# Gadersd/stable-diffusion-xl-burn

Measured on AMD Instinct MI355X. Metric: images/sec SDXL-base 1024x1024 30-step CFG7.5 (whole job); UNet step ms p50, higher is better.
Workload: dtype f16; 1 GPU; SDXL-base 1024x1024, n_steps=30 (31 CFG UNet step pairs), CFG 7.5, batch 1 prompt/GPU + VAE decode to u8 (BASELINE configs[1]); precision=f16, vae_dtype=f32_split, weights=synthetic seeded (random-init SDXL-base architecture), mix_classes=0, parallelism=replica x1, 1 prompt per GPU, weights broadcast once over RCCL, hipgraph=True, split_cfg=False, fused_xattn=True, pipelined_decode=False, prompts_per_call=1, full=False, library=stable-diffusion-xl-burn_amd/lib/libsdxl_mi355.so, debug_set=

## Files before the change

### stable-diffusion-xl-burn_amd/csrc/igemm_wreg.hip

```cpp
#include "igemm_common.h"
#include <atomic>

namespace sdxl {

template <int OFF> __device__ __forceinline__ half8 wreg_gload128(const half_t* ptr) {
  half8 v;
  asm volatile("global_load_dwordx4 %0, %1, off offset:%2" : "=v"(v) : "v"(ptr), "n"(OFF));
  return v;
}

__global__ void repack_wfrag_kernel(const f32x4* __restrict__ src, f32x4* __restrict__ dst, int nblocks, int nk) {
  const size_t i = (size_t)blockIdx.x * blockDim.x + threadIdx.x;
  const size_t total = (size_t)nblocks * nk * 256;
  if (i >= total) return;
  const int lane = (int)(i & 63), kk = (int)((i >> 6) & 3);
  const size_t t = i >> 8;
  const int kt = (int)(t % nk);
  const int nb = (int)(t / nk);
  dst[i] = src[(size_t)(nb * 32 + (lane & 31)) * (nk * 8) + kt * 8 + kk * 2 + (lane >> 5)];
}
void launch_repack_wfrag(const void* w, void* wf, int Npad, int Kpad, hipStream_t s) {
  const int nblocks = Npad / 32, nk = Kpad / 64;
  const size_t total = (size_t)nblocks * nk * 256;
  hipLaunchKernelGGL(repack_wfrag_kernel, dim3((unsigned)((total + 255) / 256)), dim3(256), 0, s, reinterpret_cast<const f32x4*>(w),
                     reinterpret_cast<f32x4*>(wf), nblocks, nk);
}

template <int TM> struct WregEpiOperands { half8 rh[TM]; f32x4 rf[TM][2]; f32x4 bz0, bz1, sg0, sg1; };
template <int TM>
__device__ __forceinline__ void wreg_epilogue_request(const IgemmParams& p, int mw, int nw, int lane, int t, const void* zeros, WregEpiOperands<TM>& op) {
  const int fr = lane & 31, fh = lane >> 5;
  const f32x4* zv = reinterpret_cast<const f32x4*>(zeros);
  const int n0 = nw + t * 16 + 8 * fh;
  const bool r16 = p.R && p.r_dt == DT_F16, r32 = p.R && p.r_dt == DT_F32;
#pragma unroll
  for (int i = 0; i < TM; ++i) {
    const int m = mw + i * 32 + fr;
    const bool ok = m < p.M;
    const size_t o = (size_t)(ok ? m : 0) * p.ldr + n0;
    op.rh[i] = *((r16 && ok) ? reinterpret_cast<const half8*>(reinterpret_cast<const half_t*>(p.R) + o) : reinterpret_cast<const half8*>(zeros));
    if (r32) {
      op.rf[i][0] = *(ok ? reinterpret_cast<const f32x4*>(reinterpret_cast<const float*>(p.R) + o) : zv);
      op.rf[i][1] = *(ok ? reinterpret_cast<const f32x4*>(reinterpret_cast<const float*>(p.R) + o + 4) : zv);
    }
  }
  op.bz0 = *(p.bias ? reinterpret_cast<const f32x4*>(p.bias + nw + 16 * t + 4 * fh) : zv);
  op.bz1 = *(p.bias ? reinterpret_cast<const f32x4*>(p.bias + nw + 16 * t + 8 + 4 * fh) : zv);
  op.sg0 = *(p.shadow ? reinterpret_cast<const f32x4*>(p.shadow_gamma + n0) : zv);
  op.sg1 = *(p.shadow ? reinterpret_cast<const f32x4*>(p.shadow_gamma + n0 + 4) : zv);
}
template <int TM>
__device__ __forceinline__ void wreg_epilogue(const IgemmParams& p, const f32x16 (&acc)[TM], int mw, int nw, int lane, int w, int t,
                                              float* xch, const WregEpiOperands<TM>& op) {
  const int fr = lane & 31, fh = lane >> 5;
  float sv[TM][8];
  int m[TM];
  bool mok[TM];
#pragma unroll
  for (int i = 0; i < TM; ++i) { m[i] = mw + i * 32 + fr; mok[i] = m[i] < p.M; }
  const int n0 = nw + t * 16 + 8 * fh;
  {
    const bool r16 = p.R && p.r_dt == DT_F16, r32 = p.R && p.r_dt == DT_F32;
    const half8 (&rh)[TM] = op.rh;
    const f32x4 (&rf)[TM][2] = op.rf;
    const f32x4 bz0 = op.bz0, bz1 = op.bz1;
#pragma unroll
    for (int i = 0; i < TM; ++i) {
      f32x4 v0, v1;
#pragma unroll
      for (int r = 0; r < 4; ++r) {
        v0[r] = t ? acc[i][8 + r] : acc[i][r];
        v1[r] = t ? acc[i][12 + r] : acc[i][4 + r];
      }
      v0 = v0 + bz0; v1 = v1 + bz1;
      float wv[8];
#pragma unroll
      for (int r = 0; r < 4; ++r) {
        const auto sw = __builtin_amdgcn_permlane32_swap(__float_as_uint(v0[r]), __float_as_uint(v1[r]), false, false);
        wv[r] = __uint_as_float(sw[0]);
        wv[4 + r] = __uint_as_float(sw[1]);
      }
      if (r16) {
#pragma unroll
        for (int e = 0; e < 8; ++e) wv[e] += (float)rh[i][e];
      } else if (r32) {
#pragma unroll
        for (int e = 0; e < 4; ++e) { wv[e] += rf[i][0][e]; wv[4 + e] += rf[i][1][e]; }
      }
      if (p.c_dt == DT_F16) {
        half8 h;
#pragma unroll
        for (int e = 0; e < 8; ++e) h[e] = (half_t)wv[e];
        if (mok[i]) *reinterpret_cast<half8*>(reinterpret_cast<half_t*>(p.C) + (size_t)m[i] * p.ldc + n0) = h;
#pragma unroll
        for (int e = 0; e < 8; ++e) sv[i][e] = (float)h[e];
      } else {
        if (mok[i]) {
          float* cp = reinterpret_cast<float*>(p.C) + (size_t)m[i] * p.ldc + n0;
          *reinterpret_cast<f32x4*>(cp) = f32x4{wv[0], wv[1], wv[2], wv[3]};
          *reinterpret_cast<f32x4*>(cp + 4) = f32x4{wv[4], wv[5], wv[6], wv[7]};
        }
        if (p.shadow && p.shadow_lo_scale < 0.f) {
          float xs[8];
#pragma unroll
          for (int e = 0; e < 4; ++e) { xs[e] = wv[e] * op.sg0[e]; xs[4 + e] = wv[4 + e] * op.sg1[e]; }
          if (mok[i]) store_hl8(reinterpret_cast<float*>(p.shadow) + (size_t)m[i] * p.shadow_ld, n0, xs);
        } else
        if (p.shadow) {
          half8 hs;
#pragma unroll
          for (int e = 0; e < 4; ++e) { hs[e] = (half_t)(wv[e] * op.sg0[e]); hs[4 + e] = (half_t)(wv[4 + e] * op.sg1[e]); }
          if (p.shadow_lo_scale > 0.f) {
            half8 hl;
#pragma unroll
            for (int e = 0; e < 4; ++e) {
              float x0 = wv[e] * op.sg0[e], x1 = wv[4 + e] * op.sg1[e];
              asm("" : "+v"(x0)); asm("" : "+v"(x1));
// ... 137 lines not shown
    xattn_unit_long(qf, op.kf, op.vf, fx, p.xa_nctx, fh, o);
  } else
  xattn_unit(qf, op.kf, op.vf, p.xa_nctx, fh, o);
  const int m = m0 + 32 * ui + fr;
  half_t* crow = reinterpret_cast<half_t*>(p.C) + (size_t)(m < p.M ? m : 0) * p.ldc + n0 + 64 * uh + 8 * fh;
#pragma unroll
  for (int dt = 0; dt < 2; ++dt)
#pragma unroll
    for (int t = 0; t < 2; ++t) {
      half8 h;
#pragma unroll
      for (int r = 0; r < 4; ++r) {
        const auto sw = __builtin_amdgcn_permlane32_swap(__float_as_uint(o[dt][8 * t + r]), __float_as_uint(o[dt][8 * t + 4 + r]), false, false);
        h[r] = (half_t)__uint_as_float(sw[0]);
        h[4 + r] = (half_t)__uint_as_float(sw[1]);
      }
      if (m < p.M) *reinterpret_cast<half8*>(crow + 32 * dt + 16 * t) = h;
    }
}

#ifdef SDXL_MEASURE
__device__ unsigned* g_wreg_tl = nullptr;
void igemm_set_wreg_timeline(void* buf) {
  unsigned* b = reinterpret_cast<unsigned*>(buf);
  if (hipMemcpyToSymbol(HIP_SYMBOL(g_wreg_tl), &b, sizeof(b)) != hipSuccess) throw std::runtime_error("igemm_wreg: cannot set the timeline buffer");
}
#define WREG_STAMP(i) do { wtl[i] = (unsigned)__builtin_amdgcn_s_memtime(); } while (0)
#else
#define WREG_STAMP(i) do { } while (0)
#endif
constexpr int wreg_mode_flags(int m) {
  return m >= 16 ? m : m == 1 ? 16 : m == 2 ? 32 : m == 3 ? 64 : m == 4 ? 128 : m == 5 ? 256 : m == 6 ? 512 : m == 7 ? 1024 : m == 8 ? 2048 : 0;
}
template <int BM, int L, int MODE = 0, int XA = 0>
__global__ __launch_bounds__(512) void igemm_wreg_kernel(const IgemmParams p, const void* zeros) {
#ifdef SDXL_MEASURE
  unsigned wtl[8] = {0, 0, 0, 0, 0, 0, 0, 0};
  wtl[6] = (unsigned)__builtin_amdgcn_s_memrealtime();
#endif
  WREG_STAMP(0);
  kernarg_prefetch<(int)sizeof(IgemmParams) + 8>();
  constexpr int NG = 2;
  constexpr int NSG = L + 1;
  constexpr int TM = BM / 32;
  constexpr int PP = BM / 32;
  constexpr int FL = wreg_mode_flags(MODE);
  constexpr bool NOMFMA = FL & 16, FROZEN = FL & 32, NOVMEM = FL & 64, NOBAR = FL & 128, XCDALT = FL & 256, NOA = FL & 512, NOWL = FL & 1024,
                 ACONTIG = FL & 2048, NOLDS = FL & 4096;
  constexpr int NW = NOWL ? 0 : 4;
  constexpr int NA = NOA ? 0 : PP;
  constexpr int U = NA + NW;
  constexpr int NOPS = U;
  constexpr int SLOT = BM * 128;
  constexpr int RING = NSG * SLOT;
  constexpr int KSTEP = 64 * NG;
  static_assert(BM % 32 == 0 && TM >= 2 && TM <= 4, "wave tile: 64 / 96 / 128 rows");
  static_assert((NSG - 1) * SLOT + (TM - 1) * 4096 < 65536, "fragment offsets must fit the ds_read immediate");
  static_assert(PP + (L - 1) * U < 64 && L >= 2, "vmcnt is 6 bits");
  static_assert(NOPS <= 3 * TM, "one VMEM operation per MFMA gap before the rendezvous");
  extern __shared__ __attribute__((aligned(16))) char smem[];
  const unsigned lds0 = (unsigned)(uintptr_t)(lptr_t)smem;

  const int tid = threadIdx.x, lane = tid & 63;
  const int wave = __builtin_amdgcn_readfirstlane(tid >> 6);
  const int g = wave >> 2, w = wave & 3;

  const int tilesM = (p.M + BM - 1) / BM;
  const int nwg = tilesM * (p.N >> 7);
  if ((int)blockIdx.x >= nwg) {
#pragma unroll
    for (int r = 0; r < 3; ++r)
      if (p.warm[r]) igemm_warm_body<512>(p.warm[r], p.warm_bytes[r], (int)blockIdx.x - nwg, (int)gridDim.x - nwg);
    return;
  }
  int bid = blockIdx.x;
  {
    const int q = nwg >> 3, r = nwg & 7, xcd = bid & 7, idx = bid >> 3;
    bid = (xcd < r ? xcd * (q + 1) : r * (q + 1) + (xcd - r) * q) + idx;
  }
  const int tilesN = p.N >> 7;
  int tm = bid / tilesN, tn = bid - tm * tilesN;
  if constexpr (XCDALT) { tn = bid / tilesM; tm = bid - tn * tilesM; }
  if (p.wreg_xcd2d && !(tilesM & 1) && !(tilesN & 1) && tilesN >= 8) {
    const int ch = tilesN >> 1, prow = tilesM >> 1, ptiles = prow * ch;
    const int patch = bid / ptiles, idx = bid - patch * ptiles;
    const int r = idx / ch;
    tm = (patch >> 1) * prow + r;
    tn = (patch & 1) * ch + (idx - r * ch);
  }
  const int m0 = tm * BM, n0 = tn * 128;
  const int nk = p.Kpad >> 6;
  const int nkg = (nk - g + 1) >> 1;

  const half_t* wp = reinterpret_cast<const half_t*>(p.Wf) + ((size_t)((n0 >> 5) + w) * nk + g) * 2048 + lane * 8;
  half8 Wr[NSG][4];
  if constexpr (NOVMEM || NOWL) { static_for<NSG>([&](auto S_) { static_for<4>([&](auto K_) { Wr[decltype(S_)::value][decltype(K_)::value] = half8{1, 1, 1, 1, 1, 1, 1, 1}; }); }); }
  auto loadW = [&](auto S, auto KK) {
    constexpr int s = decltype(S)::value, kk = decltype(KK)::value;
    if constexpr (!NOVMEM && !NOWL) Wr[s][kk] = wreg_gload128<kk * 1024>(wp);
    if constexpr (kk == 3 && !FROZEN) wp += NG * 2048;
  };
  const half_t* Ag = reinterpret_cast<const half_t*>(p.A);
  const half_t* aptr[PP];
  int aadv[PP];
  char* const ring = smem + g * RING;
  auto setupA = [&]() {
#pragma unroll
    for (int q = 0; q < PP; ++q) {
      const int row = (q * 4 + w) * 8 + (lane >> 3);
      const int m = m0 + row;
      const bool ok = m < p.M;
      aptr[q] = ok ? Ag + (size_t)m * p.lda + g * 64 + (((lane & 7) ^ ((row >> 1) & 7)) << 3) : reinterpret_cast<const half_t*>(zeros);
      aadv[q] = ok ? KSTEP : 0;
      if constexpr (ACONTIG) {
        aptr[q] = Ag + ((size_t)(tm % (p.M / BM)) * nk + g) * (BM * 64) + (q * 4 + w) * 512 + lane * 8;
        aadv[q] = NG * BM * 64;
      }
    }
  };
  auto pieceA = [&](auto S, auto Q) {
    constexpr int s = decltype(S)::value, q = decltype(Q)::value;
    if constexpr (!NOVMEM && !NOA) __builtin_amdgcn_global_load_lds((gptr_t)aptr[q], (lptr_t)(ring + s * SLOT + (q * 4 + w) * 1024), 16, 0, 0);
    if constexpr (!FROZEN) aptr[q] += aadv[q];
  };
  auto vmem_op = [&](auto S, auto X) {
    constexpr int x = decltype(X)::value;
    if constexpr (x < NW) loadW(S, X);
    else pieceA(S, std::integral_constant<int, x - NW>{});
  };

  const int fr = lane & 31, fh = lane >> 5;
  unsigned fa[4];
  {
    const unsigned basea = lds0 + g * RING + fr * 128 + ((fh ^ ((fr >> 1) & 7)) << 4);
#pragma unroll
    for (int kk = 0; kk < 4; ++kk) fa[kk] = basea ^ (kk << 5);
  }
  half8 fA[2][TM];
  if constexpr (NOLDS) { static_for<TM>([&](auto I) { fA[0][decltype(I)::value] = fA[1][decltype(I)::value] = half8{1, 1, 1, 1, 1, 1, 1, 1}; }); }
  auto ldsA = [&](auto SET, auto S, auto KK) {
    constexpr int set = decltype(SET)::value, s = decltype(S)::value, kk = decltype(KK)::value;
    if constexpr (!NOLDS) static_for<TM>([&](auto I) { fA[set][decltype(I)::value] = lds_read128<s * SLOT + decltype(I)::value * 4096>(fa[kk]); });
  };
  using I0 = std::integral_constant<int, 0>; using I1 = std::integral_constant<int, 1>;
  using I2 = std::integral_constant<int, 2>; using I3 = std::integral_constant<int, 3>;

  const int s0 = ((L - (nkg - 1)) % NSG + NSG) % NSG;
  const int ns = nkg > L ? nkg - L : 0;

  static_for<NSG>([&](auto C) {
    constexpr int c = decltype(C)::value;
    if (s0 == c && nkg > 0) static_for<4>([&](auto KK) { loadW(C, KK); });
  });
  setupA();
  static_for<NSG>([&](auto C) {
    constexpr int c = decltype(C)::value;
    if (s0 == c) {
      static_for<L>([&](auto I) {
        constexpr int i = decltype(I)::value;
        using SI = std::integral_constant<int, (c + i) % NSG>;
        if (i < nkg) {
          if constexpr (i > 0) static_for<4>([&](auto KK) { loadW(SI{}, KK); });
          static_for<PP>([&](auto Q) { pieceA(SI{}, Q); });
        }
      });
    }
  });
  __builtin_amdgcn_sched_barrier(0);
  WREG_STAMP(1);
  f32x16 acc[TM];
#pragma unroll
  for (int i = 0; i < TM; ++i)
#pragma unroll
    for (int r = 0; r < 16; ++r) acc[i][r] = 0.f;

// ... 43 lines not shown
      wait_lgkmcnt<0>();
      if constexpr (!NOBAR) __builtin_amdgcn_s_barrier();
      asm volatile("" ::: "memory");
      __builtin_amdgcn_sched_barrier(0);
      ldsA(I0{}, SN{}, I0{});
    } else {
      wait_lgkmcnt<0>();
    }
    mma(I1{}, S, I3{}, SF{}, NOX{});
  };
  using STEADY = std::integral_constant<int, 0>;
  if (ns > 0) {
    const int first = s0 == 0 ? 1 : NSG - s0 + 1;
    static_for<L>([&](auto C) { constexpr int c = decltype(C)::value + 1; if (s0 != 0 && s0 <= c) ktile(std::integral_constant<int, c>{}, STEADY{}); });
    ktile(I0{}, STEADY{});
    for (int pass = (ns - first) / NSG; pass > 0; --pass) {
      static_for<L>([&](auto C) { ktile(std::integral_constant<int, decltype(C)::value + 1>{}, STEADY{}); });
      ktile(I0{}, STEADY{});
    }
  }
  static_for<L>([&](auto X) {
    constexpr int D = L - decltype(X)::value;
    if (D <= nkg) ktile(std::integral_constant<int, L + 1 - D>{}, std::integral_constant<int, D>{});
  });
  WREG_STAMP(3);
  if constexpr (!NOBAR) { if ((nk & 1) && g == 1) __builtin_amdgcn_s_barrier(); }
  asm volatile("" ::: "memory");
  __builtin_amdgcn_sched_barrier(0);

  WregEpiOperands<TM> eop;
  WregXaOperands<XA ? BM : 64> xop;
  float* const xa_coef = reinterpret_cast<float*>(smem + NG * RING);
  if constexpr (XA) { static_assert(MODE == 0, "production arithmetic only"); wreg_xattn_request<BM, XA == 2>(p, m0, n0, lane, wave, zeros, xop); }
  else wreg_epilogue_request<TM>(p, m0, n0 + w * 32, lane, g, zeros, eop);
  static_assert(4 * TM * 2 * 64 * 16 <= L * SLOT, "a group's four exchange pieces must fit its dead slots 0 .. L - 1");
  f32x4* xw = reinterpret_cast<f32x4*>(smem + g * RING) + (size_t)w * (TM * 2 * 64) + lane;
  const f32x4* xo = reinterpret_cast<const f32x4*>(smem + (1 - g) * RING) + (size_t)w * (TM * 2 * 64) + lane;
#pragma unroll
  for (int i = 0; i < TM; ++i)
#pragma unroll
    for (int qq = 0; qq < 2; ++qq) {
      f32x4 v;
#pragma unroll
      for (int r = 0; r < 4; ++r) v[r] = g ? acc[i][4 * qq + r] : acc[i][8 + 4 * qq + r];
      xw[(i * 2 + qq) * 64] = v;
    }
  if constexpr (XA) wreg_xattn_coef<BM>(p, m0, lane, wave, xop, xa_coef);
  wait_lgkmcnt<0>();
  __builtin_amdgcn_s_barrier();
  asm volatile("" ::: "memory");
#pragma unroll
  for (int i = 0; i < TM; ++i)
#pragma unroll
    for (int qq = 0; qq < 2; ++qq) {
      const f32x4 o = xo[(i * 2 + qq) * 64];
#pragma unroll
      for (int r = 0; r < 4; ++r) {
        if (g) acc[i][8 + 4 * qq + r] = o[r] + acc[i][8 + 4 * qq + r];
        else acc[i][4 * qq + r] = acc[i][4 * qq + r] + o[r];
      }
    }
  WREG_STAMP(4);
  static_assert((2 * BM + 6 * 2 * BM) * 4 <= SLOT, "statistics exchange must fit one slot");
  float* xch = reinterpret_cast<float*>(smem + L * SLOT);
  if constexpr (XA) wreg_xattn_tail<BM, L, XA == 2>(p, acc, m0, n0, lane, wave, smem, xa_coef, xop);
  else wreg_epilogue<TM>(p, acc, m0, n0 + w * 32, lane, w, g, xch, eop);
#ifdef SDXL_MEASURE
  WREG_STAMP(5);
  asm volatile("s_waitcnt vmcnt(0)" ::: "memory");
  wtl[7] = (unsigned)__builtin_amdgcn_s_memrealtime();
  { const unsigned t6 = (unsigned)__builtin_amdgcn_s_memtime();
    if (g_wreg_tl && lane == 0) { unsigned* d = g_wreg_tl + ((size_t)blockIdx.x * 8 + wave) * 16; for (int i = 0; i < 8; ++i) d[i] = wtl[i]; d[8] = t6; } }
#endif
}

static std::atomic<int> g_wreg_xcd2d{0};
void igemm_set_wreg_xcd2d(int v) { g_wreg_xcd2d = v; }
static std::atomic<int> g_warm_enable{1};
void igemm_set_warm(int v) { g_warm_enable = v; }
int igemm_warm_enabled() { return g_warm_enable.load(); }

template <int BM, int L, int MODE = 0, int XA = 0>
static void launch_wreg_t(const IgemmParams& p, const IgemmChoice& c, hipStream_t s) {
  constexpr size_t lds = (size_t)2 * (L + 1) * BM * 128 + (XA ? BM * 8 : 0);
  static_assert(lds >= (size_t)8 * (BM / 32) * 2048 + (size_t)(2 * BM + 6 * 2 * BM) * 4, "exchange areas must fit the dead rings");
  if ((size_t)c.lds != lds) throw std::logic_error("igemm_wreg: choice and kernel disagree on the LDS layout");
  set_max_dynamic_lds<&igemm_wreg_kernel<BM, L, MODE, XA>>(lds, igemm_current_device());
  IgemmParams q = p;
  q.wreg_xcd2d = g_wreg_xcd2d.load();
  hipLaunchKernelGGL((igemm_wreg_kernel<BM, L, MODE, XA>), dim3(c.grid), dim3(c.block), lds, s, q, igemm_zero_page());
}

void launch_igemm_wreg(const IgemmParams& p, const IgemmChoice& c, hipStream_t s) {
#define WREG(BM, L, MODE, XA) \
  if (c.bm == BM && c.ns == L && c.mode == (MODE) && (c.xa > 1 ? 2 : c.xa) == XA) return launch_wreg_t<BM, L, (MODE), XA>(p, c, s)
#ifdef SDXL_MEASURE
  WREG(96, 3, 0, 0); WREG(96, 4, 0, 0); WREG(128, 2, 0, 0);
  WREG(96, 2, 1, 0); WREG(96, 2, 2, 0); WREG(96, 2, 3, 0); WREG(96, 2, 4, 0); WREG(96, 2, 5, 0);
  WREG(96, 2, 6, 0); WREG(96, 2, 7, 0); WREG(96, 2, 8, 0);
  WREG(96, 2, 16 | 32, 0); WREG(96, 2, 16 | 32 | 4096, 0); WREG(96, 2, 16 | 32 | 4096 | 128, 0); WREG(96, 2, 16 | 4096, 0); WREG(96, 2, 4096, 0);
#endif
  WREG(64, 2, 0, 0); WREG(96, 2, 0, 0);
  WREG(64, 2, 0, 1); WREG(96, 2, 0, 1);
  WREG(64, 2, 0, 2); WREG(96, 2, 0, 2);
#undef WREG
  throw std::logic_error("igemm_wreg: the selection chose a kernel that is not instantiated");
}

}
```

### stable-diffusion-xl-burn_amd/csrc/select.cpp

```cpp
#include "kernels.h"
#include <algorithm>
#include <atomic>
#include <cstring>
#include <stdexcept>

namespace sdxl {

namespace {
struct KnobSlot { const char* key; int SelectKnobs::*field; };
constexpr KnobSlot kKnobSlots[] = {
    {"igemm_variant", &SelectKnobs::igemm_variant}, {"igemm_wreg", &SelectKnobs::igemm_wreg}, {"wreg_xattn", &SelectKnobs::wreg_xattn},
    {"hl_tile96", &SelectKnobs::hl_tile96},         {"igemm_tsw", &SelectKnobs::igemm_tsw},   {"wide_db", &SelectKnobs::wide_db},
    {"attn_variant", &SelectKnobs::attn_variant},   {"attn_xsplit", &SelectKnobs::attn_xsplit},
#ifdef SDXL_MEASURE
    {"igemm_unrolled", &SelectKnobs::igemm_unrolled},
#endif
};
constexpr int kNumKnobs = sizeof(kKnobSlots) / sizeof(kKnobSlots[0]);
struct KnobStore {
  std::atomic<int> v[kNumKnobs];
  KnobStore() { const SelectKnobs d; for (int i = 0; i < kNumKnobs; ++i) v[i] = d.*kKnobSlots[i].field; }
};
KnobStore g_knobs;
}
// ... 70 lines not shown
  if (p.ph_rows <= 0 || p.ph_wbytes == 0 || p.B <= 0 || p.ph_rows != p.B * p.Hin * p.Win || p.M != 4 * p.ph_rows) return false;
  if (p.ksize != 2 || p.stride != 1 || p.up != 0 || p.pad != 1 || p.Hout != p.Hin || p.Wout != p.Win) return false;
  if ((p.Hin * p.Win) % 128 != 0 || p.Cin % kt != 0 || p.K != 4 * p.Cin || p.Kpad != p.K) return false;
  return p.act == 0 && p.n_split >= p.N && !p.R && !p.ebias && !p.stat_out && !p.gn_part && !p.ln_stat && !p.xa_k && !p.shadow;
}
int pick_phase_tile(const IgemmParams& p, int nk, bool hl) {
  double best = 1e300;
  int number = 36;
  for (int n : {35, 36, 38, 49}) {
    const Tile& t = tile(n);
    if (p.ph_rows % t.bm != 0 || !tile_takes(t, p) || (hl && n == 38)) continue;
    const double cost = tile_cost(p.M, p.N, nk, t.bm, t.bn, t.w);
    if (cost < best) { best = cost; number = n; }
  }
  if (!hl && number == 36 && nk >= 40) number = 44;
  return number;
}

struct Fill { long t96, t128, t256; double eff128, eff256; };
Fill chip_fill(const IgemmParams& p) {
  const long cols = (p.N + 127) / 128;
  const long t96 = (long)((p.M + 95) / 96) * cols, t128 = (long)((p.M + 127) / 128) * cols, t256 = (long)((p.M + 255) / 256) * cols;
  return {t96, t128, t256, (double)t128 / (double)(((t128 + 255) / 256) * 256), (double)t256 / (double)(((t256 + 255) / 256) * 256)};
}
int fill_tile_256_or_128(const IgemmParams& p) {
  const Fill f = chip_fill(p);
  return f.eff256 >= f.eff128 ? 35 : 36;
}

bool wreg_pair_grid_fits(const IgemmParams& p) {
  const long rows = 2L * (p.rpb > 0 ? p.rpb : p.M);
  return ((rows + 95) / 96) * (long)(p.N / 128) <= 512;
}
int wreg_rows(const IgemmParams& p) { return (long)((p.M + 63) / 64) * (p.N / 128) <= 256 ? 64 : 96; }
bool wreg_takes(const IgemmParams& p, const SelectKnobs& k, bool xa) {
  if (!p.Wf || !k.zero_page || (xa ? !p.xa_k || p.xa_k_lo : p.xa_k != nullptr)) return false;
  if (p.a_dt != DT_F16 || (p.c_dt != DT_F16 && (xa || p.c_dt != DT_F32))) return false;
  if (p.ksize != 1 || p.stride != 1 || p.up != 0 || p.pad != 0 || p.Hin != p.Hout || p.Win != p.Wout) return false;
  if (p.N % 128 != 0 || p.Cin != p.K || p.K != p.Kpad || p.Kpad % 64 != 0 || p.Kpad < 128) return false;
  if (p.act != 0 || p.n_split < p.N || p.gn_part || p.acc_scale || p.ebias) return false;
  if ((p.lda & 7) != 0 || misaligned16(p.A) || (p.ldc & 7) != 0 || misaligned16(p.C)) return false;
  if (xa) {
    if (p.stat_out || p.R || p.shadow || p.rpb <= 0 || p.rpb % 64 != 0 || p.M % p.rpb != 0 || p.xa_nctx < 1) return false;
    return p.xa_nctx <= 96 || igemm_xattn_ok(p.a_dt, p.c_dt, p.M, p.N, p.K, p.rpb, p.xa_nctx, k, true);
  }
  if (p.ln_stat || (p.R && ((p.ldr & 7) != 0 || misaligned16(p.R)))) return false;
  if (p.shadow && (p.c_dt != DT_F32 || !p.shadow_gamma || (p.shadow_ld & (p.shadow_lo_scale < 0.f ? 15 : 7)) != 0 || misaligned16(p.shadow))) return false;
  return true;
}
#ifdef SDXL_MEASURE
struct WregForced { int number, bm, depth, mode; };
constexpr WregForced kWregForced[] = {{61, 128, 2, 0}, {63, 96, 2, 1}, {64, 96, 2, 2}, {65, 96, 2, 3}, {66, 96, 2, 4}, {67, 96, 2, 5}, {68, 96, 3, 0},
    {69, 96, 4, 0}, {70, 96, 2, 6}, {71, 96, 2, 7}, {72, 96, 2, 8}, {73, 96, 2, 16 | 32}, {74, 96, 2, 16 | 32 | 4096}, {75, 96, 2, 16 | 32 | 4096 | 128},
    {76, 96, 2, 16 | 4096}, {77, 96, 2, 4096}};
#endif

void set_geometry(IgemmChoice& c, const IgemmParams& p) {
  const int tilesM = (p.M + c.bm - 1) / c.bm, tilesN = (p.N + c.bn - 1) / c.bn;
  c.grid = tilesM * tilesN * (c.splitk > 1 ? c.splitk : 1);
  switch (c.family) {
    case IG_GLDS: c.block = 256; c.lds = c.ns * (c.bm + c.bn) * 128; break;
    case IG_PIPE: {
      const int ring = c.ns * (c.bm + c.bn) * 128;
      c.block = 64 * c.nw; c.lds = ring + 2048 <= 163840 ? ring + 2048 : ring;
    } break;
    case IG_WIDE: c.block = 512; c.lds = c.ns * (c.bm + c.bn) * 64 + 2048; break;
    case IG_WREG: {
      int warm = 0;
      if (p.warm[0] && p.warm_bytes[0] && c.grid <= 512) {
        const int spare = (c.grid <= 256 ? 256 : 512) - c.grid;
        warm = spare < 8 ? 0 : spare > 64 ? 64 : spare;
      }
      c.grid += warm;
      c.block = 512; c.lds = 2 * (c.ns + 1) * c.bm * 128 + (c.xa ? c.bm * 8 : 0);
    } break;
    case IG_GENERIC: c.block = 256; c.lds = 2 * (c.bm + c.bn) * 128; break;
    default: break;
  }
}
IgemmChoice from_tile(int number, int elem, const IgemmParams& p) {
  const Tile& t = tile(number);
  IgemmChoice c{};
  c.family = t.family; c.bm = t.bm; c.bn = t.bn; c.ns = t.ns; c.wgm = t.wgm; c.nw = t.nw; c.s2 = t.s2; c.elem = elem; c.a_elem = elem; c.splitk = 1;
  set_geometry(c, p);
  return c;
}
IgemmChoice wreg_choice(int bm, int depth, int mode, bool xa, const IgemmParams& p) {
  IgemmChoice c{};
  c.family = IG_WREG; c.bm = bm; c.bn = 128; c.ns = depth; c.nw = 8; c.mode = mode; c.elem = c.a_elem = DT_F16; c.splitk = 1;
  c.xa = xa ? (p.xa_nctx + 95) / 96 : 0;
  set_geometry(c, p);
  return c;
}
IgemmChoice wreg_forced_or_auto(int v, bool xa, const IgemmParams& p) {
#ifdef SDXL_MEASURE
  if (!xa) for (const WregForced& f : kWregForced) if (f.number == v) return wreg_choice(f.bm, f.depth, f.mode, false, p);
#endif
  return wreg_choice(v == 60 ? 96 : v == 62 ? 64 : wreg_rows(p), 2, 0, xa, p);
}

bool select_f16(const IgemmParams& p, int v, const SelectKnobs& k, IgemmChoice& c) {
  if (!k.zero_page) return false;
  if (p.act > 1) return false;
  if (p.a_dt != DT_F16 || (p.Cin % 64) != 0 || (p.lda % 8) != 0 || (p.Kpad % 64) != 0) return false;
  if (misaligned16(p.A)) return false;
  if (p.n_split < p.N && (p.n_split & 3) != 0) return false;
  if (p.ebias && (p.ebias_ld & 3) != 0) return false;
  if (p.stat_out && (v == 2 || v == 5 || v == 19 || v == 38)) return false;
  const bool was_auto = v == 0;
  const int nk = p.Kpad / 64;
  if (p.ph_rows) {
    if (!phase_shape_ok(p, 64)) throw std::runtime_error("igemm: the phase form of an upsample convolution was given a launch it does not take");
    c = from_tile(pick_phase_tile(p, nk, false), DT_F16, p);
    return true;
  }
  if (p.xa_k) {
    if (p.act != 0 || p.n_split < p.N || p.stat_out || p.R || p.ebias ||
        !igemm_xattn_ok(p.a_dt, p.c_dt, p.M, p.N, p.K, p.rpb, p.xa_nctx, k, p.Wf && !p.xa_k_lo))
      throw std::runtime_error("igemm: fused cross-attention needs a plain f16 projection (no residual / split outputs)");
    if (!p.xa_k_lo && p.c_dt != DT_F16) throw std::runtime_error("igemm: the f16 fused cross-attention writes f16 rows");
    const bool forced_pipe = xattn_forced_pipe(v);
    if (p.xa_nctx > 96 && (forced_pipe || !igemm_wreg_xattn_selected(p, k)))
      throw std::runtime_error("igemm: fused cross-attention over more than 96 keys needs the weights-in-registers kernel");
    if (p.xa_k_lo) {
      c = from_tile(pick_tile(p, {36, 45}) == 45 ? 45 : 36, DT_F16, p);
      c.xh = 1;
      if (c.bm == 96) c.ns = 3;
    } else if (!forced_pipe && igemm_wreg_xattn_selected(p, k)) {
      c = wreg_forced_or_auto(v, true, p);
      return true;
    } else {
      c = from_tile(forced_pipe ? v : pick_tile(p, {35, 36, 45}), DT_F16, p);
      if (c.bm == 96) c.ns = 3;
    }
    c.xa = 1;
    set_geometry(c, p);
    return true;
  }
  if (p.gn_part) {
    if (!igemm_gn_part_ok(p, k)) throw std::runtime_error("igemm: GroupNorm statistics requested from a shape the 256x128 epilogue does not take");
    v = 0;
  }
  if (p.shadow) {
    if (!igemm_wreg_selected(p, k)) throw std::runtime_error("igemm: an f16 shadow output needs the weights-in-registers kernel");
    c = wreg_forced_or_auto(0, false, p);
    return true;
  }
  if (v == 0 ? igemm_wreg_selected(p, k) : (v >= 60 && v <= 77 && wreg_takes(p, k, false))) { c = wreg_forced_or_auto(v, false, p); return true; }
  if (v >= 60 && v <= 77) return false;
  if (v == 0 && igemm_splitk_slices(p) > 1) {
    c = from_tile(35, DT_F16, p);
    c.splitk = igemm_splitk_slices(p);
    set_geometry(c, p);
    return true;
  }
  if (v == 0) v = p.gn_part ? 35 : pick_tile(p, {35, 36, 45, 38, 49, 26});
#ifdef SDXL_MEASURE
  if (was_auto && !k.igemm_unrolled) {
    if (v == 35) v = 11; else if (v == 36) v = 13; else if (v == 38) v = 19;
  }
#else
  (void)was_auto;
#endif
  const Tile* t = find_tile(v);
  if (!t) {
#ifdef SDXL_MEASURE
    c = IgemmChoice{}; c.family = IG_MEASURE; c.measure = v; c.splitk = 1;
    return true;
#else
    return false;
#endif
  }
  if (!tile_takes(*t, p)) return false;
  c = from_tile(v, DT_F16, p);
  if (v == 35 && p.n_split < p.N && k.igemm_tsw && p.c_dt == DT_F16) c.tsw = 1;
#ifdef SDXL_MEASURE
  if (c.family == IG_WIDE) c.db = k.wide_db != 0;
#endif
  return true;
}

bool select_f32(const IgemmParams& p, const SelectKnobs& k, IgemmChoice& c) {
// ... 50 lines not shown

IgemmChoice select_generic(const IgemmParams& p, int compute_dt) {
  struct Cand { int bm, bn; float eff; };
  const Cand cands[4] = {{128, 128, 1.0f}, {128, 64, 0.85f}, {64, 128, 0.85f}, {64, 64, 0.70f}};
  int best = 0; float best_cost = 1e30f;
  for (int i = 0; i < 4; ++i) {
    if (p.act == 1 && cands[i].bn < 64) continue;
    const long tiles = (long)((p.M + cands[i].bm - 1) / cands[i].bm) * ((p.N + cands[i].bn - 1) / cands[i].bn);
    const int slots = 256 * (cands[i].bm * cands[i].bn >= 128 * 128 ? 2 : 4);
    const long waves = (tiles + slots - 1) / slots;
    const float cost = (float)waves * cands[i].bm * cands[i].bn / cands[i].eff;
    if (cost < best_cost) { best_cost = cost; best = i; }
  }
  IgemmChoice c{};
  c.family = IG_GENERIC; c.bm = cands[best].bm; c.bn = cands[best].bn; c.ns = 2; c.wgm = 2; c.nw = 4; c.splitk = 1;
  c.elem = compute_dt == DT_F16 ? DT_F16 : DT_F32;
  c.a_elem = compute_dt == DT_F16 && p.a_dt == DT_F16 ? DT_F16 : DT_F32;
  set_geometry(c, p);
  return c;
}
}

int igemm_splitk_slices(const IgemmParams& p) {
  if (!p.splitk_ws || !p.splitk_cnt) return 1;
  if (p.act != 0 || p.n_split < p.N || p.ln_stat) return 1;
  const int nk = p.Kpad / 64;
  if (p.rpb <= 0 || p.rpb > 1024 || p.N > 1536 || nk < 160) return 1;
  return p.rpb <= 256 ? 8 : 3;
}
size_t igemm_splitk_ws_bytes(int batch, int rows_per_entry, int n_max) {
  if (n_max > 1536) n_max = 1536;
  const long rows3 = (long)batch * (rows_per_entry < 1024 ? rows_per_entry : 1024), rows8 = (long)batch * (rows_per_entry < 256 ? rows_per_entry : 256);
  const size_t slabs3 = (size_t)((rows3 + 255) / 256) * 3, slabs8 = (size_t)((rows8 + 255) / 256) * 8;
  return (slabs3 > slabs8 ? slabs3 : slabs8) * (size_t)((n_max + 127) / 128) * 256 * 128 * 4;
}

bool igemm_gn_part_ok(const IgemmParams& p, const SelectKnobs& k) {
  const bool hl = p.a_dt == DT_HL;
  const int kt = hl ? 32 : 64;
  if (hl ? p.c_dt != DT_F32 : (p.a_dt != DT_F16 || p.c_dt != DT_F16)) return false;
  if ((p.Cin % kt) != 0 || (p.lda % (kt / 8)) != 0 || (p.Kpad % kt) != 0) return false;
  if (p.act != 0 || p.n_split < p.N || p.stat_out || p.ln_stat || p.xa_k) return false;
  if (p.M % 256 != 0 || p.rpb <= 0 || p.rpb % 256 != 0 || p.N % 64 != 0) return false;
  if (p.ebias && (p.ebias_ld & 3) != 0) return false;
  if (hl) return (p.ldc & 3) == 0 && !misaligned16(p.C) && (k.hl_tile96 & 16) && igemm_splitk_slices(p) > 1;
  if (igemm_splitk_slices(p) > 1) return true;
  IgemmParams q = p;
  q.M = 2 * p.rpb;
  if (pick_tile(q, {35, 36, 45, 38, 26}) != 35) return false;
  const int nk = p.Kpad / 64;
  return p.N % 160 != 0 || tile_cost(q, nk, 35) - tile_cost(q, nk, 49) < 6000.0;
}

bool igemm_xattn_ok(int a_dt, int c_dt, int M, int N, int K, int rpb, int n_ctx, const SelectKnobs& k, bool wreg_form) {
  if (!(a_dt == DT_F16 && (c_dt == DT_F16 || c_dt == DT_HL) && M > 0 && N % 64 == 0 && K % 64 == 0 && rpb > 0 && rpb % 64 == 0 && M % rpb == 0 && n_ctx >= 1))
    return false;
  if (n_ctx <= 96) return true;
  if (!wreg_form || n_ctx > 96 * xattn_long_max_blocks || c_dt != DT_F16 || N % 128 != 0 || K < 128) return false;
  if (!k.zero_page || !k.igemm_wreg || !k.wreg_xattn || k.igemm_variant < 0 || xattn_forced_pipe(k.igemm_variant)) return false;
  IgemmParams q{};
  q.M = M; q.N = N; q.rpb = rpb;
  return wreg_pair_grid_fits(q);
}
bool igemm_phase_ok(const IgemmParams& p, int compute_dt, const SelectKnobs& k) {
  if (k.igemm_variant < 0 || !phase_shape_ok(p, compute_dt == DT_HL ? 32 : 64)) return false;
  IgemmChoice c{};
  return compute_dt == DT_F16 ? select_f16(p, 0, k, c) : (compute_dt == DT_HL && select_hl(p, k, c));
// ... 82 lines not shown
```

Measured before the change: 1.502 images/sec.

## Add 192-row tall tile and two-way split-K to weights-in-registers GEMM

```diff
diff --git a/stable-diffusion-xl-burn_amd/csrc/igemm_wreg.hip b/stable-diffusion-xl-burn_amd/csrc/igemm_wreg.hip
--- a/stable-diffusion-xl-burn_amd/csrc/igemm_wreg.hip
+++ b/stable-diffusion-xl-burn_amd/csrc/igemm_wreg.hip
@@ -26,7 +26,16 @@
                      reinterpret_cast<f32x4*>(wf), nblocks, nk);
 }
 
-template <int TM> struct WregEpiOperands { half8 rh[TM]; f32x4 rf[TM][2]; f32x4 bz0, bz1, sg0, sg1; };
+template <int TM> struct WregEpiOperands {
+  half8 rh[TM]; f32x4 rf[TM][2]; f32x4 bz0, bz1, sg0, sg1;
+  __device__ __forceinline__ void set_rh(int i, half8 v) { rh[i] = v; }
+  __device__ __forceinline__ half8 get_rh(int i) const { return rh[i]; }
+};
+template <> struct WregEpiOperands<6> {
+  f32x4 rf[6][2]; f32x4 bz0, bz1, sg0, sg1;
+  __device__ __forceinline__ void set_rh(int i, half8 v) { rf[i][0] = __builtin_bit_cast(f32x4, v); }
+  __device__ __forceinline__ half8 get_rh(int i) const { return __builtin_bit_cast(half8, rf[i][0]); }
+};
 template <int TM>
 __device__ __forceinline__ void wreg_epilogue_request(const IgemmParams& p, int mw, int nw, int lane, int t, const void* zeros, WregEpiOperands<TM>& op) {
   const int fr = lane & 31, fh = lane >> 5;
@@ -38,7 +47,7 @@
     const int m = mw + i * 32 + fr;
     const bool ok = m < p.M;
     const size_t o = (size_t)(ok ? m : 0) * p.ldr + n0;
-    op.rh[i] = *((r16 && ok) ? reinterpret_cast<const half8*>(reinterpret_cast<const half_t*>(p.R) + o) : reinterpret_cast<const half8*>(zeros));
+    op.set_rh(i, *((r16 && ok) ? reinterpret_cast<const half8*>(reinterpret_cast<const half_t*>(p.R) + o) : reinterpret_cast<const half8*>(zeros)));
     if (r32) {
       op.rf[i][0] = *(ok ? reinterpret_cast<const f32x4*>(reinterpret_cast<const float*>(p.R) + o) : zv);
       op.rf[i][1] = *(ok ? reinterpret_cast<const f32x4*>(reinterpret_cast<const float*>(p.R) + o + 4) : zv);
@@ -61,7 +70,6 @@
   const int n0 = nw + t * 16 + 8 * fh;
   {
     const bool r16 = p.R && p.r_dt == DT_F16, r32 = p.R && p.r_dt == DT_F32;
-    const half8 (&rh)[TM] = op.rh;
     const f32x4 (&rf)[TM][2] = op.rf;
     const f32x4 bz0 = op.bz0, bz1 = op.bz1;
 #pragma unroll
@@ -81,8 +89,9 @@
         wv[4 + r] = __uint_as_float(sw[1]);
       }
       if (r16) {
-#pragma unroll
-        for (int e = 0; e < 8; ++e) wv[e] += (float)rh[i][e];
+        const half8 rh = op.get_rh(i);
+#pragma unroll
+        for (int e = 0; e < 8; ++e) wv[e] += (float)rh[e];
       } else if (r32) {
 #pragma unroll
         for (int e = 0; e < 4; ++e) { wv[e] += rf[i][0][e]; wv[4 + e] += rf[i][1][e]; }
@@ -286,7 +295,7 @@
 constexpr int wreg_mode_flags(int m) {
   return m >= 16 ? m : m == 1 ? 16 : m == 2 ? 32 : m == 3 ? 64 : m == 4 ? 128 : m == 5 ? 256 : m == 6 ? 512 : m == 7 ? 1024 : m == 8 ? 2048 : 0;
 }
-template <int BM, int L, int MODE = 0, int XA = 0>
+template <int BM, int L, int MODE = 0, int XA = 0, int SK = 1>
 __global__ __launch_bounds__(512) void igemm_wreg_kernel(const IgemmParams p, const void* zeros) {
 #ifdef SDXL_MEASURE
   unsigned wtl[8] = {0, 0, 0, 0, 0, 0, 0, 0};
@@ -308,8 +317,11 @@
   constexpr int SLOT = BM * 128;
   constexpr int RING = NSG * SLOT;
   constexpr int KSTEP = 64 * NG;
-  static_assert(BM % 32 == 0 && TM >= 2 && TM <= 4, "wave tile: 64 / 96 / 128 rows");
-  static_assert((NSG - 1) * SLOT + (TM - 1) * 4096 < 65536, "fragment offsets must fit the ds_read immediate");
+  static_assert(BM % 32 == 0 && TM >= 2 && (TM <= 4 || TM == 6), "wave tile: 64 / 96 / 128 / 192 rows");
+  static_assert(TM <= 4 || (XA == 0 && MODE == 0), "192 rows: plain form only");
+  static_assert(SK == 1 || (SK == 2 && XA == 0 && MODE == 0), "k-slices: two, plain form only");
+  constexpr int FRAG_HI = 32768;
+  static_assert((NSG - 1) * SLOT + (TM - 1) * 4096 < 65536 + FRAG_HI, "fragment offsets must fit the ds_read immediate");
   static_assert(PP + (L - 1) * U < 64 && L >= 2, "vmcnt is 6 bits");
   static_assert(NOPS <= 3 * TM, "one VMEM operation per MFMA gap before the rendezvous");
   extern __shared__ __attribute__((aligned(16))) char smem[];
@@ -320,7 +332,8 @@
   const int g = wave >> 2, w = wave & 3;
 
   const int tilesM = (p.M + BM - 1) / BM;
-  const int nwg = tilesM * (p.N >> 7);
+  const int ntile = tilesM * (p.N >> 7);
+  const int nwg = ntile * SK;
   if ((int)blockIdx.x >= nwg) {
 #pragma unroll
     for (int r = 0; r < 3; ++r)
@@ -332,6 +345,8 @@
     const int q = nwg >> 3, r = nwg & 7, xcd = bid & 7, idx = bid >> 3;
     bid = (xcd < r ? xcd * (q + 1) : r * (q + 1) + (xcd - r) * q) + idx;
   }
+  int slice = 0;
+  if constexpr (SK > 1) { slice = bid >= ntile ? 1 : 0; bid -= slice * ntile; }
   const int tilesN = p.N >> 7;
   int tm = bid / tilesN, tn = bid - tm * tilesN;
   if constexpr (XCDALT) { tn = bid / tilesM; tm = bid - tn * tilesM; }
@@ -343,10 +358,12 @@
     tn = (patch & 1) * ch + (idx - r * ch);
   }
   const int m0 = tm * BM, n0 = tn * 128;
-  const int nk = p.Kpad >> 6;
+  const int nk_all = p.Kpad >> 6;
+  const int kt0 = SK > 1 && slice ? (nk_all + 1) >> 1 : 0;
+  const int nk = SK > 1 ? (slice ? nk_all - kt0 : (nk_all + 1) >> 1) : nk_all;
   const int nkg = (nk - g + 1) >> 1;
 
-  const half_t* wp = reinterpret_cast<const half_t*>(p.Wf) + ((size_t)((n0 >> 5) + w) * nk + g) * 2048 + lane * 8;
+  const half_t* wp = reinterpret_cast<const half_t*>(p.Wf) + ((size_t)((n0 >> 5) + w) * nk_all + kt0 + g) * 2048 + lane * 8;
   half8 Wr[NSG][4];
   if constexpr (NOVMEM || NOWL) { static_for<NSG>([&](auto S_) { static_for<4>([&](auto K_) { Wr[decltype(S_)::value][decltype(K_)::value] = half8{1, 1, 1, 1, 1, 1, 1, 1}; }); }); }
   auto loadW = [&](auto S, auto KK) {
@@ -355,8 +372,11 @@
     if constexpr (kk == 3 && !FROZEN) wp += NG * 2048;
   };
   const half_t* Ag = reinterpret_cast<const half_t*>(p.A);
-  const half_t* aptr[PP];
-  int aadv[PP];
+  constexpr bool TALL = BM == 192;
+  const half_t* aptr[TALL ? 1 : PP];
+  int aadv[TALL ? 1 : PP];
+  unsigned aoff[TALL ? PP : 1];
+  const char* const abase = reinterpret_cast<const char*>(Ag + (kt0 + g) * 64);
   char* const ring = smem + g * RING;
   auto setupA = [&]() {
 #pragma unroll
@@ -364,18 +384,27 @@
       const int row = (q * 4 + w) * 8 + (lane >> 3);
       const int m = m0 + row;
       const bool ok = m < p.M;
-      aptr[q] = ok ? Ag + (size_t)m * p.lda + g * 64 + (((lane & 7) ^ ((row >> 1) & 7)) << 3) : reinterpret_cast<const half_t*>(zeros);
+      if constexpr (TALL) {
+        aoff[q] = ((unsigned)(ok ? m : p.M - 1) * (unsigned)p.lda + (unsigned)(((lane & 7) ^ ((row >> 1) & 7)) << 3)) * 2u;
+      } else {
+      aptr[q] = ok ? Ag + (size_t)m * p.lda + (kt0 + g) * 64 + (((lane & 7) ^ ((row >> 1) & 7)) << 3) : reinterpret_cast<const half_t*>(zeros);
       aadv[q] = ok ? KSTEP : 0;
       if constexpr (ACONTIG) {
         aptr[q] = Ag + ((size_t)(tm % (p.M / BM)) * nk + g) * (BM * 64) + (q * 4 + w) * 512 + lane * 8;
         aadv[q] = NG * BM * 64;
       }
+      }
     }
   };
   auto pieceA = [&](auto S, auto Q) {
     constexpr int s = decltype(S)::value, q = decltype(Q)::value;
+    if constexpr (TALL) {
+      __builtin_amdgcn_global_load_lds((gptr_t)(abase + aoff[q]), (lptr_t)(ring + s * SLOT + (q * 4 + w) * 1024), 16, 0, 0);
+      aoff[q] += KSTEP * 2;
+    } else {
     if constexpr (!NOVMEM && !NOA) __builtin_amdgcn_global_load_lds((gptr_t)aptr[q], (lptr_t)(ring + s * SLOT + (q * 4 + w) * 1024), 16, 0, 0);
     if constexpr (!FROZEN) aptr[q] += aadv[q];
+    }
   };
   auto vmem_op = [&](auto S, auto X) {
     constexpr int x = decltype(X)::value;
@@ -385,16 +414,23 @@
 
   const int fr = lane & 31, fh = lane >> 5;
   unsigned fa[4];
-  {
-    const unsigned basea = lds0 + g * RING + fr * 128 + ((fh ^ ((fr >> 1) & 7)) << 4);
-#pragma unroll
-    for (int kk = 0; kk < 4; ++kk) fa[kk] = basea ^ (kk << 5);
-  }
+  const unsigned basea = lds0 + g * RING + fr * 128 + ((fh ^ ((fr >> 1) & 7)) << 4);
+#pragma unroll
+  for (int kk = 0; kk < 4; ++kk) fa[kk] = basea ^ (kk << 5);
   half8 fA[2][TM];
   if constexpr (NOLDS) { static_for<TM>([&](auto I) { fA[0][decltype(I)::value] = fA[1][decltype(I)::value] = half8{1, 1, 1, 1, 1, 1, 1, 1}; }); }
   auto ldsA = [&](auto SET, auto S, auto KK) {
     constexpr int set = decltype(SET)::value, s = decltype(S)::value, kk = decltype(KK)::value;
-    if constexpr (!NOLDS) static_for<TM>([&](auto I) { fA[set][decltype(I)::value] = lds_read128<s * SLOT + decltype(I)::value * 4096>(fa[kk]); });
+    unsigned a = fa[kk];
+    if constexpr (TALL) {
+      a = basea;
+      asm volatile("" : "+v"(a));
+      a ^= kk << 5;
+    }
+    if constexpr (!NOLDS) static_for<TM>([&](auto I) {
+      constexpr int off = s * SLOT + decltype(I)::value * 4096, hi = off >= 65536 ? FRAG_HI : 0;
+      fA[set][decltype(I)::value] = lds_read128<off - hi>(a + hi);
+    });
   };
   using I0 = std::integral_constant<int, 0>; using I1 = std::integral_constant<int, 1>;
   using I2 = std::integral_constant<int, 2>; using I3 = std::integral_constant<int, 3>;
@@ -504,7 +540,7 @@
   WregXaOperands<XA ? BM : 64> xop;
   float* const xa_coef = reinterpret_cast<float*>(smem + NG * RING);
   if constexpr (XA) { static_assert(MODE == 0, "production arithmetic only"); wreg_xattn_request<BM, XA == 2>(p, m0, n0, lane, wave, zeros, xop); }
-  else wreg_epilogue_request<TM>(p, m0, n0 + w * 32, lane, g, zeros, eop);
+  else if constexpr (SK == 1) wreg_epilogue_request<TM>(p, m0, n0 + w * 32, lane, g, zeros, eop);
   static_assert(4 * TM * 2 * 64 * 16 <= L * SLOT, "a group's four exchange pieces must fit its dead slots 0 .. L - 1");
   f32x4* xw = reinterpret_cast<f32x4*>(smem + g * RING) + (size_t)w * (TM * 2 * 64) + lane;
   const f32x4* xo = reinterpret_cast<const f32x4*>(smem + (1 - g) * RING) + (size_t)w * (TM * 2 * 64) + lane;
@@ -532,6 +568,53 @@
         else acc[i][4 * qq + r] = acc[i][4 * qq + r] + o[r];
       }
     }
+  if constexpr (SK > 1) {
+    constexpr int NV = TM * 2;
+    const int tile_id = tm * tilesN + tn;
+    f32x4* const slabs = reinterpret_cast<f32x4*>(p.splitk_ws) + (size_t)tile_id * 2 * (size_t)(8 * NV * 64) + (size_t)(wave * NV * 64 + lane);
+    f32x4* const mine = slabs + (size_t)slice * (8 * NV * 64);
+#pragma unroll
+    for (int i = 0; i < TM; ++i)
+#pragma unroll
+      for (int qq = 0; qq < 2; ++qq) {
+        f32x4 v;
+#pragma unroll
+        for (int r = 0; r < 4; ++r) v[r] = g ? acc[i][8 + 4 * qq + r] : acc[i][4 * qq + r];
+        f32x4* dst = mine + (i * 2 + qq) * 64;
+        if (p.splitk_wt) asm volatile("global_store_dwordx4 %0, %1, off sc0 sc1\n\ts_nop 1" ::"v"(dst), "v"(v) : "memory");
+        else *dst = v;
+      }
+    asm volatile("s_waitcnt vmcnt(0)" ::: "memory");
+    __syncthreads();
+    volatile int* flag = reinterpret_cast<volatile int*>(smem + L * SLOT + SLOT - 16);
+    if (tid == 0) {
+      if (!p.splitk_wt) __builtin_amdgcn_fence(__ATOMIC_RELEASE, "agent");
+      asm volatile("s_waitcnt vmcnt(0)" ::: "memory");
+      const unsigned t = __hip_atomic_fetch_add(p.splitk_cnt + tile_id, 1u, __ATOMIC_RELAXED, __HIP_MEMORY_SCOPE_AGENT);
+      const int last = t == 1u;
+      if (last) {
+        __hip_atomic_store(p.splitk_cnt + tile_id, 0u, __ATOMIC_RELAXED, __HIP_MEMORY_SCOPE_AGENT);
+        __builtin_amdgcn_fence(__ATOMIC_ACQUIRE, "agent");
+      }
+      *flag = last;
+    }
+    __syncthreads();
+    if (!*flag) return;
+    wreg_epilogue_request<TM>(p, m0, n0 + w * 32, lane, g, zeros, eop);
+    const f32x4* const other = slabs + (size_t)(1 - slice) * (8 * NV * 64);
+#pragma unroll
+    for (int i = 0; i < TM; ++i)
+#pragma unroll
+      for (int qq = 0; qq < 2; ++qq) {
+        const f32x4 o = other[(i * 2 + qq) * 64];
+#pragma unroll
+        for (int r = 0; r < 4; ++r) {
+          const float a = g ? acc[i][8 + 4 * qq + r] : acc[i][4 * qq + r];
+          const float sum = slice ? o[r] + a : a + o[r];
+          if (g) acc[i][8 + 4 * qq + r] = sum; else acc[i][4 * qq + r] = sum;
+        }
+      }
+  }
   WREG_STAMP(4);
   static_assert((2 * BM + 6 * 2 * BM) * 4 <= SLOT, "statistics exchange must fit one slot");
   float* xch = reinterpret_cast<float*>(smem + L * SLOT);
@@ -552,20 +635,30 @@
 void igemm_set_warm(int v) { g_warm_enable = v; }
 int igemm_warm_enabled() { return g_warm_enable.load(); }
 
-template <int BM, int L, int MODE = 0, int XA = 0>
+template <int BM, int L, int MODE = 0, int XA = 0, int SK = 1>
 static void launch_wreg_t(const IgemmParams& p, const IgemmChoice& c, hipStream_t s) {
   constexpr size_t lds = (size_t)2 * (L + 1) * BM * 128 + (XA ? BM * 8 : 0);
   static_assert(lds >= (size_t)8 * (BM / 32) * 2048 + (size_t)(2 * BM + 6 * 2 * BM) * 4, "exchange areas must fit the dead rings");
   if ((size_t)c.lds != lds) throw std::logic_error("igemm_wreg: choice and kernel disagree on the LDS layout");
-  set_max_dynamic_lds<&igemm_wreg_kernel<BM, L, MODE, XA>>(lds, igemm_current_device());
   IgemmParams q = p;
+  if constexpr (SK > 1) {
+    const size_t tiles = (size_t)((p.M + BM - 1) / BM) * (size_t)(p.N / 128);
+    if (!p.splitk_ws || !p.splitk_cnt || tiles * 2 * BM * 128 * 4 > p.splitk_ws_bytes) throw std::runtime_error("igemm_wreg: split-K workspace too small");
+    if (tiles > (size_t)kSplitkCounters) throw std::runtime_error("igemm_wreg: more tiles than split-K counters");
+    if (p.Kpad < 256) throw std::logic_error("igemm_wreg: a k-slice needs two k-tiles");
+  }
+  set_max_dynamic_lds<&igemm_wreg_kernel<BM, L, MODE, XA, SK>>(lds, igemm_current_device());
   q.wreg_xcd2d = g_wreg_xcd2d.load();
-  hipLaunchKernelGGL((igemm_wreg_kernel<BM, L, MODE, XA>), dim3(c.grid), dim3(c.block), lds, s, q, igemm_zero_page());
+  hipLaunchKernelGGL((igemm_wreg_kernel<BM, L, MODE, XA, SK>), dim3(c.grid), dim3(c.block), lds, s, q, igemm_zero_page());
 }
 
 void launch_igemm_wreg(const IgemmParams& p, const IgemmChoice& c, hipStream_t s) {
 #define WREG(BM, L, MODE, XA) \
-  if (c.bm == BM && c.ns == L && c.mode == (MODE) && (c.xa > 1 ? 2 : c.xa) == XA) return launch_wreg_t<BM, L, (MODE), XA>(p, c, s)
+  if (c.bm == BM && c.ns == L && c.mode == (MODE) && (c.xa > 1 ? 2 : c.xa) == XA && c.splitk <= 1) return launch_wreg_t<BM, L, (MODE), XA>(p, c, s)
+#define WREG_SK(BM) \
+  if (c.bm == BM && c.ns == 2 && c.mode == 0 && c.xa == 0 && c.splitk == 2) return launch_wreg_t<BM, 2, 0, 0, 2>(p, c, s)
+  WREG(192, 2, 0, 0); WREG_SK(192); WREG_SK(96); WREG_SK(64);
+#undef WREG_SK
 #ifdef SDXL_MEASURE
   WREG(96, 3, 0, 0); WREG(96, 4, 0, 0); WREG(128, 2, 0, 0);
   WREG(96, 2, 1, 0); WREG(96, 2, 2, 0); WREG(96, 2, 3, 0); WREG(96, 2, 4, 0); WREG(96, 2, 5, 0);
diff --git a/stable-diffusion-xl-burn_amd/csrc/select.cpp b/stable-diffusion-xl-burn_amd/csrc/select.cpp
--- a/stable-diffusion-xl-burn_amd/csrc/select.cpp
+++ b/stable-diffusion-xl-burn_amd/csrc/select.cpp
@@ -126,7 +126,20 @@
   const long rows = 2L * (p.rpb > 0 ? p.rpb : p.M);
   return ((rows + 95) / 96) * (long)(p.N / 128) <= 512;
 }
-int wreg_rows(const IgemmParams& p) { return (long)((p.M + 63) / 64) * (p.N / 128) <= 256 ? 64 : 96; }
+constexpr bool kWregSliceAuto = false;
+bool wreg_slices_ok(const IgemmParams& p) { return p.splitk_ws && p.splitk_cnt && p.Kpad >= 256 && !p.xa_k; }
+bool wreg_sliced_layer(const IgemmParams& p) { return kWregSliceAuto && wreg_slices_ok(p) && p.N == 1280 && p.Kpad >= 5120; }
+bool wreg_tall_ok(const IgemmParams& p) { return !p.xa_k && (long long)p.M * p.lda * 2 < (1LL << 31); }
+int wreg_rows(const IgemmParams& p, bool sliced = false) {
+  const long cols = p.N / 128;
+  if (!sliced) {
+    const long t96 = (long)((p.M + 95) / 96) * cols, t192 = (long)((p.M + 191) / 192) * cols;
+    if (wreg_tall_ok(p) && p.N == 640 && p.Kpad >= 2560 && ((t192 + 255) / 256) * 2 <= (t96 + 255) / 256) return 192;
+    return (long)((p.M + 63) / 64) * cols <= 256 ? 64 : 96;
+  }
+  if ((long)((p.M + 63) / 64) * cols * 2 <= 256) return 64;
+  return (long)((p.M + 95) / 96) * cols * 2 <= 256 ? 96 : 192;
+}
 bool wreg_takes(const IgemmParams& p, const SelectKnobs& k, bool xa) {
   if (!p.Wf || !k.zero_page || (xa ? !p.xa_k || p.xa_k_lo : p.xa_k != nullptr)) return false;
   if (p.a_dt != DT_F16 || (p.c_dt != DT_F16 && (xa || p.c_dt != DT_F32))) return false;
@@ -149,6 +162,8 @@
     {76, 96, 2, 16 | 4096}, {77, 96, 2, 4096}};
 #endif
 
+struct WregTall { int number, bm, slices; };
+constexpr WregTall kWregTall[] = {{78, 192, 0}, {79, 192, 1}, {80, 96, 1}, {81, 64, 1}};
 void set_geometry(IgemmChoice& c, const IgemmParams& p) {
   const int tilesM = (p.M + c.bm - 1) / c.bm, tilesN = (p.N + c.bn - 1) / c.bn;
   c.grid = tilesM * tilesN * (c.splitk > 1 ? c.splitk : 1);
@@ -161,7 +176,7 @@
     case IG_WIDE: c.block = 512; c.lds = c.ns * (c.bm + c.bn) * 64 + 2048; break;
     case IG_WREG: {
       int warm = 0;
-      if (p.warm[0] && p.warm_bytes[0] && c.grid <= 512) {
+      if (p.warm[0] && p.warm_bytes[0] && c.grid <= (c.bm == 192 ? 256 : 512)) {
         const int spare = (c.grid <= 256 ? 256 : 512) - c.grid;
         warm = spare < 8 ? 0 : spare > 64 ? 64 : spare;
       }
@@ -179,9 +194,9 @@
   set_geometry(c, p);
   return c;
 }
-IgemmChoice wreg_choice(int bm, int depth, int mode, bool xa, const IgemmParams& p) {
+IgemmChoice wreg_choice(int bm, int depth, int mode, bool xa, const IgemmParams& p, bool sliced = false) {
   IgemmChoice c{};
-  c.family = IG_WREG; c.bm = bm; c.bn = 128; c.ns = depth; c.nw = 8; c.mode = mode; c.elem = c.a_elem = DT_F16; c.splitk = 1;
+  c.family = IG_WREG; c.bm = bm; c.bn = 128; c.ns = depth; c.nw = 8; c.mode = mode; c.elem = c.a_elem = DT_F16; c.splitk = sliced ? 2 : 1;
   c.xa = xa ? (p.xa_nctx + 95) / 96 : 0;
   set_geometry(c, p);
   return c;
@@ -190,7 +205,13 @@
 #ifdef SDXL_MEASURE
   if (!xa) for (const WregForced& f : kWregForced) if (f.number == v) return wreg_choice(f.bm, f.depth, f.mode, false, p);
 #endif
-  return wreg_choice(v == 60 ? 96 : v == 62 ? 64 : wreg_rows(p), 2, 0, xa, p);
+  bool sliced = !xa && wreg_sliced_layer(p);
+  int bm = 0;
+  if (!xa) for (const WregTall& f : kWregTall) if (f.number == v) { bm = f.bm; sliced = sliced || (f.slices && wreg_slices_ok(p)); }
+  if (v == 60) bm = 96; else if (v == 62) bm = 64;
+  if (bm == 0) bm = wreg_rows(p, sliced);
+  if (bm == 192 && !wreg_tall_ok(p)) bm = 96;
+  return wreg_choice(bm, 2, 0, xa, p, sliced);
 }
 
 bool select_f16(const IgemmParams& p, int v, const SelectKnobs& k, IgemmChoice& c) {
@@ -237,11 +258,11 @@
   }
   if (p.shadow) {
     if (!igemm_wreg_selected(p, k)) throw std::runtime_error("igemm: an f16 shadow output needs the weights-in-registers kernel");
-    c = wreg_forced_or_auto(0, false, p);
-    return true;
-  }
-  if (v == 0 ? igemm_wreg_selected(p, k) : (v >= 60 && v <= 77 && wreg_takes(p, k, false))) { c = wreg_forced_or_auto(v, false, p); return true; }
-  if (v >= 60 && v <= 77) return false;
+    c = wreg_forced_or_auto(v >= 78 && v <= 81 ? v : 0, false, p);
+    return true;
+  }
+  if (v == 0 ? igemm_wreg_selected(p, k) : (v >= 60 && v <= 81 && wreg_takes(p, k, false))) { c = wreg_forced_or_auto(v, false, p); return true; }
+  if (v >= 60 && v <= 81) return false;
   if (v == 0 && igemm_splitk_slices(p) > 1) {
     c = from_tile(35, DT_F16, p);
     c.splitk = igemm_splitk_slices(p);
@@ -358,7 +379,9 @@
   if (n_max > 1536) n_max = 1536;
   const long rows3 = (long)batch * (rows_per_entry < 1024 ? rows_per_entry : 1024), rows8 = (long)batch * (rows_per_entry < 256 ? rows_per_entry : 256);
   const size_t slabs3 = (size_t)((rows3 + 255) / 256) * 3, slabs8 = (size_t)((rows8 + 255) / 256) * 8;
-  return (slabs3 > slabs8 ? slabs3 : slabs8) * (size_t)((n_max + 127) / 128) * 256 * 128 * 4;
+  const size_t pipe = (slabs3 > slabs8 ? slabs3 : slabs8) * (size_t)((n_max + 127) / 128) * 256 * 128 * 4;
+  const size_t wreg = n_max >= 1280 ? ((size_t)batch * rows_per_entry + 191) * 1280 * 4 * 2 : 0;
+  return pipe > wreg ? pipe : wreg;
 }
 
 bool igemm_gn_part_ok(const IgemmParams& p, const SelectKnobs& k) {
```

Result: no change. 1.498 images/sec (-0.3%).
